# meffmadd/intro-tc-vae

Measured on AMD Instinct MI355X. Metric: images/sec (64x64x3, z=128, bs=64) intro-TC step, higher is better.
Workload: dtype f32 in/out/accumulate, conv products on split-fp16 MFMA (two scaled fp16 planes, 3 products, fp32-class)

## Files before the change

include/itcv_hip.h:

```cpp
#ifndef ITCV_HIP_H
#define ITCV_HIP_H

#include <stddef.h>
#include <stdint.h>

#ifdef __cplusplus
extern "C" {
#endif

#define ITCV_ABI_VERSION 4

int itcv_abi_version(void);
const char* itcv_last_error(void);
int itcv_set_option(const char* name, int value);
int itcv_get_option(const char* name);

int itcv_profile_begin(void);
int itcv_profile_end(void);
int itcv_profile_get(int i, int* code, double* flop, float* ms);
int itcv_profile_clear(void);

size_t itcv_conv2d_packed_weight_elems(int Co, int Ci, int KS, int for_dgrad);
int itcv_conv2d_pack_weight(const float* w, float* wp, int Co, int Ci, int KS, int for_dgrad,
                            void* stream);
// ... 93 lines not shown
                     void* stream);
int itcv_bn_finalize_uv(const double* sums, double count, float eps, float momentum, float* running_mean,
                        float* running_var, int64_t* num_batches_tracked, float* mean, float* rstd, float* unbiased_var,
                        int C, void* stream);
int itcv_bn_eval_stats(const float* running_mean, const float* running_var, float eps, float* mean,
                       float* rstd, int C, void* stream);
int itcv_bn_act_fwd(const float* x, const float* mean, const float* rstd, const float* gamma,
                    const float* beta, const float* skip, float* y, int B, int C, int H, int W,
                    float slope, int pool, void* planes, int ns, size_t plane_stride, void* stream);
int itcv_bn_act_planes_supported(int C, int H, int W, int pool);
int itcv_bn_act_bwd_reduce(const float* x, const float* dy, const float* mean, const float* rstd,
                           const float* gamma, const float* beta, const float* skip, double* dsums,
                           float* dgamma, float* dbeta, int accumulate, int B, int C, int H, int W,
                           float slope, int pool, int up2, void* ws, size_t ws_bytes, void* stream);
int itcv_bn_act_bwd_apply(const float* x, const float* dy, const float* mean, const float* rstd,
                          const float* gamma, const float* beta, const float* skip, const double* dsums,
                          const double* local_dsums, double count, float* dx, float* dskip,
                          float* dgamma, float* dbeta, int accumulate, int B, int C, int H, int W,
                          float slope, int pool, int up2, void* dx_planes, int ns, size_t plane_stride, void* stream);

int itcv_bn_train_fwd(const float* x, const float* gamma, const float* beta, const float* skip, float* y, void* planes,
                      int ns, int B, int C, int H, int W, float slope, int pool, float eps, float momentum,
                      float* running_mean, float* running_var, int64_t* num_batches_tracked, float* mean, float* rstd,
                      void* ws, size_t ws_bytes, size_t plane_stride, const float* tile_stats, int tiles, int tile_pitch,
                      int groups, void* stream);
int itcv_bn_train_fwd_uv(const float* x, const float* gamma, const float* beta, const float* skip, float* y, void* planes,
                         int ns, int B, int C, int H, int W, float slope, int pool, float eps, float momentum,
                         float* running_mean, float* running_var, int64_t* num_batches_tracked, float* mean, float* rstd,
                         float* unbiased_var, void* ws, size_t ws_bytes, size_t plane_stride, const float* tile_stats,
                         int tiles, int tile_pitch, int groups, void* stream);
size_t itcv_bn_replay_desc_bytes(void);
int itcv_bn_replay_desc(void* host_desc, float* running_mean, float* running_var, int64_t* num_batches_tracked,
                        const float* mean, const float* unbiased_var, int C, int groups, float momentum, int block0);
int itcv_bn_replay_many(const void* dev_table, int n, int total_blocks, void* stream);
int itcv_bn_replay_max_descs(void);
int itcv_bn_train_bwd(const float* x, const float* dy, const float* mean, const float* rstd, const float* gamma,
                      const float* beta, const float* skip, double* dsums, float* dx, float* dskip, void* dx_planes,
                      int ns, float* dgamma, float* dbeta, int accumulate, int B, int C, int H, int W, float slope,
                      int pool, int up2, void* ws, size_t ws_bytes, size_t plane_stride, int groups, void* stream);
int itcv_bn_train_bwd_live(const float* x, const float* dy, const float* mean, const float* rstd, const float* gamma,
                           const float* beta, const float* skip, double* dsums, float* dx, float* dskip, void* dx_planes,
                           int ns, float* dgamma, float* dbeta, int accumulate, int B, int C, int H, int W, float slope,
                           int pool, int up2, void* ws, size_t ws_bytes, size_t plane_stride, int groups, int live0,
                           int nlive, void* stream);

#define ITCV_BN_PATH_ONE_BLOCK 0
#define ITCV_BN_PATH_SLICED_FOLD 1
#define ITCV_BN_PATH_SLICED_COMBINE 2
#define ITCV_BN_PATH_FALLBACK 3
#define ITCV_BN_PATH_PER_GROUP 4
#define ITCV_BN_PATH_TILE_STATS 5
int itcv_bn_plan_query(int bwd, int B, int C, int H, int W, int pool, int up2, int groups, int planes, int ns,
                       size_t ws_bytes, int tile_stats, int* path, int* splits);

int itcv_lrelu_fwd(const float* x, float* y, size_t n, float slope, void* stream);
int itcv_lrelu_bwd(const float* x, const float* dy, float* dx, size_t n, float slope, void* stream);
int itcv_sigmoid_fwd(const float* x, float* y, size_t n, void* stream);
int itcv_sigmoid_bwd(const float* y, const float* dy, float* dx, size_t n, void* stream);
int itcv_avgpool2_fwd(const float* x, float* y, int BC, int H, int W, void* stream);
int itcv_avgpool2_bwd(const float* dy, float* dx, int BC, int H, int W, void* stream);
int itcv_upsample2_fwd(const float* x, float* y, int BC, int H, int W, void* stream);
int itcv_upsample2_bwd(const float* dy, float* dx, int BC, int H, int W, void* stream);
int itcv_add(const float* a, const float* b, float* out, size_t n, void* stream);

int itcv_reparam_fwd(const float* mu, const float* logvar, const float* eps, float* z, size_t n,
                     void* stream);
int itcv_reparam_bwd(const float* dz, const float* logvar, const float* eps, float* dmu, float* dlogvar,
                     size_t n, void* stream);
int itcv_kl_rows_fwd(const float* logvar, const float* mu, float* kl, int B, int D, void* stream);
int itcv_kl_rows_bwd(const float* g, const float* logvar, const float* mu, float* dlogvar, float* dmu,
                     int B, int D, void* stream);

#define ITCV_TC_VAR_FROM_ROW 0x1
#define ITCV_TC_EPS_DENSITY 0x2
#define ITCV_TC_WEIGHTED 0x4
#define ITCV_TC_LIVE (ITCV_TC_VAR_FROM_ROW | ITCV_TC_EPS_DENSITY)
size_t itcv_tc_fwd_workspace(int Bl, int Bt, int D);
int itcv_tc_fwd(const float* z, const float* mu_all, const float* logvar, float* prodm, float* logqz,
                float* lse, float* sjoint, int Bl, int Bt, int row_offset, int D, int64_t dataset_size, int flags,
                void* ws, size_t ws_bytes, void* stream);
size_t itcv_tc_bwd_workspace(int Bl, int Bt);
int itcv_tc_bwd(const float* g, const float* z, const float* mu_all, const float* logvar,
                const float* logqz, const float* lse, const float* sjoint, float* dz, float* dmu_all,
                float* dlogvar, int Bl, int Bt, int row_offset, int D, int64_t dataset_size, int flags, void* ws,
                size_t ws_bytes, void* stream);
int itcv_tc_kl_fwd(const float* z, const float* mu_all, const float* logvar, float* out, float* rows, float* prodm,
                   float* logqz, float* lse, float* sjoint, int Bl, int Bt, int row_offset, int D, int64_t dataset_size,
                   float coef_tc, float coef_kl, int reduction, void* ws, size_t ws_bytes, void* stream);
int itcv_tc_kl_bwd(const float* g, const float* z, const float* mu_all, const float* logvar, const float* logqz,
                   const float* lse, const float* sjoint, float* dz, float* dmu_all, float* dlogvar, int Bl, int Bt,
                   int row_offset, int D, int64_t dataset_size, float coef_tc, float coef_kl, int reduction, void* ws,
                   size_t ws_bytes, void* stream);
size_t itcv_tc_full_fwd_workspace(int Bl, int Bt, int D);
int itcv_tc_full_fwd(const float* z, const float* mu_all, const float* logvar_all, int ld, float* out, float* rows,
                     float* comps, float* prodm, float* logqz, float* lse, float* sjoint, float* ivar, int Bl, int Bt,
                     int row_offset, int D, int64_t dataset_size, float alpha, float beta, float gamma, int reduction,
                     void* ws, size_t ws_bytes, void* stream);
size_t itcv_tc_full_bwd_workspace(int Bl, int Bt);
int itcv_tc_full_bwd(const float* g, const float* z, const float* mu_all, const float* logvar_all, int ld,
                     const float* logqz, const float* lse, const float* sjoint, const float* ivar, float* dz, float* dmu_all,
                     float* dlogvar_all, int Bl, int Bt, int row_offset, int D, int64_t dataset_size, float alpha,
                     float beta, float gamma, int reduction, void* ws, size_t ws_bytes, void* stream);
int itcv_kl_loss_fwd(const float* logvar, const float* mu, float* out, int B, int D, int reduction, float scale, void* stream);
int itcv_kl_loss_bwd(const float* g, const float* logvar, const float* mu, float* dlogvar, float* dmu, int B, int D,
                     int reduction, float scale, void* stream);
size_t itcv_dip_kl_workspace(int Bt, int D);
// ... 267 lines not shown
```

intro-tc-vae_amd/csrc/abi.hip:

```cpp
#include "conv_shared.h"

#include <vector>

namespace itcv {
thread_local char g_err[512] = "";

struct ProfRec {
  int code;
  double flop;
  hipEvent_t start, stop;
};
static bool g_prof_on = false;
static std::vector<ProfRec> g_prof;

static thread_local int g_prof_depth = 0;
ProfScope::ProfScope(hipStream_t stream, ProfKind kind, int ks, int bm, int up2, int ns, double flop) : st(stream), slot(-1) {
  if (++g_prof_depth > 1 || !g_prof_on) return;
  ProfRec r;
  r.code = kind | (ks << 4) | (bm << 8) | (up2 << 16) | (ns << 20);
  r.flop = flop;
  if (hipEventCreate(&r.start) != hipSuccess || hipEventCreate(&r.stop) != hipSuccess) return;
  g_prof.push_back(r);
  slot = (int)g_prof.size() - 1;
  g_prof_start = r.start, g_prof_stop = r.stop;
}
ProfScope::~ProfScope() {
  if (--g_prof_depth > 0) return;
  if (slot >= 0 && g_prof_start) {
    (void)hipEventDestroy(g_prof[slot].start);
    (void)hipEventDestroy(g_prof[slot].stop);
    g_prof.pop_back();
  }
  g_prof_start = g_prof_stop = nullptr;
}
thread_local hipEvent_t g_prof_start = nullptr, g_prof_stop = nullptr;
Options g_opt;
extern int g_sw_lds_rows, g_sw_max_blocks;
}

extern "C" {
int itcv_abi_version(void) { return ITCV_ABI_VERSION; }

int itcv_set_option(const char* name, int value) {
  if (!name) return itcv::fail("%s: null option name", "itcv_set_option");
  if (!strcmp(name, "band_m16")) {
    if (value != 0 && value != 1) return itcv::fail("%s: band_m16 takes 0 or 1 (got %lld)", "itcv_set_option", value);
    itcv::g_opt.band_m16 = value;
    return 0;
  }
  if (!strcmp(name, "band_persist_blocks")) {
    if (value < 0 || value > 1024) return itcv::fail("%s: band_persist_blocks takes 0..1024 (got %lld)", "itcv_set_option", value);
    itcv::g_opt.band_persist_blocks = value;
    return 0;
  }
  if (!strcmp(name, "wgrad_m16")) {
    if (value != 0 && value != 1) return itcv::fail("%s: wgrad_m16 takes 0 or 1 (got %lld)", "itcv_set_option", value);
    itcv::g_opt.wgrad_m16 = value;
    return 0;
  }
  if (!strcmp(name, "planes_mfma_waves")) {
    if (value != 4 && value != 8) return itcv::fail("%s: planes_mfma_waves takes 4 or 8 (got %lld)", "itcv_set_option", value);
    itcv::g_opt.planes_mfma_waves = value;
    return 0;
  }
  if (!strcmp(name, "sw_lds_rows")) {
    if (value < 0 || value > 4096) return itcv::fail("%s: sw_lds_rows takes 0..4096 (got %lld)", "itcv_set_option", value);
    itcv::g_sw_lds_rows = value;
    return 0;
  }
  if (!strcmp(name, "sw_max_blocks")) {
    if (value < 0 || value > 1024) return itcv::fail("%s: sw_max_blocks takes 0..1024 (got %lld)", "itcv_set_option", value);
    itcv::g_sw_max_blocks = value;
    return 0;
  }
  return itcv::fail("%s: unknown option", "itcv_set_option");
}
int itcv_get_option(const char* name) {
  if (name && !strcmp(name, "band_m16")) return itcv::g_opt.band_m16;
  if (name && !strcmp(name, "band_persist_blocks")) return itcv::g_opt.band_persist_blocks;
  if (name && !strcmp(name, "wgrad_m16")) return itcv::g_opt.wgrad_m16;
  if (name && !strcmp(name, "planes_mfma_waves")) return itcv::g_opt.planes_mfma_waves;
  if (name && !strcmp(name, "sw_lds_rows")) return itcv::g_sw_lds_rows;
  if (name && !strcmp(name, "sw_max_blocks")) return itcv::g_sw_max_blocks;
  return -1;
}
const char* itcv_last_error(void) { return itcv::g_err; }

int itcv_profile_begin(void) {
  itcv::g_prof.clear();
  itcv::g_prof_on = true;
  return 0;
}
int itcv_profile_end(void) {
  itcv::g_prof_on = false;
  for (auto& r : itcv::g_prof) (void)hipEventSynchronize(r.stop);
  return (int)itcv::g_prof.size();
}
int itcv_profile_get(int i, int* code, double* flop, float* ms) {
  if (i < 0 || i >= (int)itcv::g_prof.size()) return itcv::fail("%s: index out of range", "itcv_profile_get");
  const auto& r = itcv::g_prof[i];
  *code = r.code;
  *flop = r.flop;
  if (hipEventElapsedTime(ms, r.start, r.stop) != hipSuccess) *ms = -1.f;
  return 0;
}
int itcv_profile_clear(void) {
  for (auto& r : itcv::g_prof) {
    (void)hipEventDestroy(r.start);
    (void)hipEventDestroy(r.stop);
  }
  itcv::g_prof.clear();
  return 0;
}
}
```

intro-tc-vae_amd/csrc/norm_act.hip:

```cpp
#include <stdlib.h>

#include <type_traits>

#include "common.h"

namespace itcv {

constexpr int kRedThreads = 256;

__device__ __forceinline__ uint32_t fdiv(uint32_t a, uint32_t d, int sh) { return sh >= 0 ? (a >> sh) : (a / d); }

struct BnGrp {
  size_t xs;
  size_t os;
  size_t dys;
  size_t ps;
  int cs;
  int G;
  int lv0, lvn;
};
__device__ __forceinline__ bool bn_dead(const BnGrp& g, uint32_t group) {
  return g.lvn > 0 && (group < (uint32_t)g.lv0 || group >= (uint32_t)(g.lv0 + g.lvn));
}

// ... 335 lines not shown
      const float mu = p_mu[j], rs = p_rs[j];
      const float sc = p_ga[j] * rs, sh = p_be[j] - mu * sc;
      const size_t bc = (size_t)b * C + c;
      if (POOL == 0) {
        const size_t i = bc * HW + (size_t)pp * 4;
        float4 v = xin[POOL ? 0 : j];
        v.x = v.x * sc + sh, v.y = v.y * sc + sh, v.z = v.z * sc + sh, v.w = v.w * sc + sh;
        if (skip) {
          const float4 k = *reinterpret_cast<const float4*>(skip + i);
          v.x += k.x, v.y += k.y, v.z += k.z, v.w += k.w;
        }
        v.x = lrelu(v.x, slope), v.y = lrelu(v.y, slope), v.z = lrelu(v.z, slope), v.w = lrelu(v.w, slope);
        if (y) *reinterpret_cast<float4*>(y + i) = v;
        o[j][0] = v.x, o[j][1] = v.y, o[j][POOL ? 0 : 2] = v.z, o[j][POOL ? 1 : 3] = v.w;
      } else {
        const uint32_t ho = (pp * 2) / Wo, wo = pp * 2 - ho * Wo;
        const size_t src = bc * HW + (size_t)(2 * ho) * W + 2 * wo;
        const float4 a = *reinterpret_cast<const float4*>(x + src);
        const float4 bb = *reinterpret_cast<const float4*>(x + src + W);
        float v0 = a.x * sc + sh, v1 = a.y * sc + sh, v2 = bb.x * sc + sh, v3 = bb.y * sc + sh;
        float w0 = a.z * sc + sh, w1 = a.w * sc + sh, w2 = bb.z * sc + sh, w3 = bb.w * sc + sh;
        if (skip) {
          const float4 ka = *reinterpret_cast<const float4*>(skip + src);
          const float4 kb = *reinterpret_cast<const float4*>(skip + src + W);
          v0 += ka.x, v1 += ka.y, v2 += kb.x, v3 += kb.y;
          w0 += ka.z, w1 += ka.w, w2 += kb.z, w3 += kb.w;
        }
        const float r0 = 0.25f * (lrelu(v0, slope) + lrelu(v1, slope) + lrelu(v2, slope) + lrelu(v3, slope));
        const float r1 = 0.25f * (lrelu(w0, slope) + lrelu(w1, slope) + lrelu(w2, slope) + lrelu(w3, slope));
        if (y) *reinterpret_cast<float2*>(y + bc * HWo + (size_t)pp * 2) = make_float2(r0, r1);
        o[j][0] = r0, o[j][1] = r1;
      }
    }
    u32x4 chk[PX][NS];
#pragma unroll
    for (int px = 0; px < PX; ++px) {
      float v8[8];
#pragma unroll
      for (int j = 0; j < 8; ++j) v8[j] = o[j][px];
      split8<NS, F16>(v8, chk[px]);
    }
    const uint32_t cidx0 = base + (threadIdx.x & ~63u);
    if (cidx0 + 64 <= total) {
      store_planes_wave<PX, NS>(planes, plane_stride, per_plane, (uint32_t)HWo, cidx0, chk, strips[threadIdx.x >> 6]);
    } else {
#pragma unroll
      for (int px = 0; px < PX; ++px)
#pragma unroll
        for (int p = 0; p < NS; ++p) planes[(size_t)p * plane_stride + (size_t)bc8 * HWo + (size_t)pp * PX + px] = chk[px][p];
    }
  }
}

template <int MODE>
__device__ __forceinline__ float upstream(const float* __restrict__ dy, size_t bc, int h, int w, int H, int W) {
  if (MODE == 0) return dy[bc * H * W + (size_t)h * W + w];
  if (MODE == 1) return 0.25f * dy[bc * (H / 2) * (W / 2) + (size_t)(h >> 1) * (W / 2) + (w >> 1)];
  const size_t base = bc * (size_t)(4 * H * W) + (size_t)(2 * h) * (2 * W) + 2 * w;
  const float2 a = *reinterpret_cast<const float2*>(dy + base);
  const float2 b = *reinterpret_cast<const float2*>(dy + base + 2 * W);
  return (a.x + a.y) + (b.x + b.y);
}

template <int MODE>
__global__ __launch_bounds__(kRedThreads) void bn_bwd_partial(const float* __restrict__ x,
                                                              const float* __restrict__ dy,
                                                              const float* __restrict__ mean,
                                                              const float* __restrict__ rstd,
                                                              const float* __restrict__ gamma,
                                                              const float* __restrict__ beta,
                                                              const float* __restrict__ skip,
                                                              double* __restrict__ part, int B, int C, int H, int W,
                                                              float slope, int splits) {
  __shared__ double scratch[kRedThreads / 64];
  const int c = blockIdx.x, s = blockIdx.y, HW = H * W;
  const size_t total = (size_t)B * HW;
  const size_t chunk = (total + splits - 1) / splits;
  const size_t beg = (size_t)s * chunk, end = beg + chunk < total ? beg + chunk : total;
  const float mu = mean[c], rs = rstd[c], ga = gamma[c], be = beta[c];
  double s1 = 0.0, s2 = 0.0;
  for (size_t i = beg + threadIdx.x; i < end; i += kRedThreads) {
    const size_t b = i / HW;
    const int hw = (int)(i - b * HW), h = hw / W, w = hw - h * W;
    const size_t bc = b * C + c;
    const float xh = (x[bc * HW + hw] - mu) * rs;
    float u = xh * ga + be;
    if (skip) u += skip[bc * HW + hw];
    float g = upstream<MODE>(dy, bc, h, w, H, W);
    if (!(u > 0.f)) g *= slope;
    s1 += (double)g;
    s2 += (double)g * (double)xh;
  }
  s1 = block_sum(s1, scratch);
  s2 = block_sum(s2, scratch);
  if (threadIdx.x == 0) {
    part[((size_t)s * 2 + 0) * C + c] = s1;
    part[((size_t)s * 2 + 1) * C + c] = s2;
  }
}

template <int MODE>
__global__ void bn_bwd_apply_kernel(const float* __restrict__ x, const float* __restrict__ dy,
                                    const float* __restrict__ mean, const float* __restrict__ rstd,
                                    const float* __restrict__ gamma, const float* __restrict__ beta,
                                    const float* __restrict__ skip, const double* __restrict__ dsums, double count,
                                    float* __restrict__ dx, float* __restrict__ dskip, int C, int H, int W,
// ... 503 lines not shown
}

static inline int bn_fmt(int ns) { return ns == ITCV_PLANES_F16X2 ? 2 : (ns == 2 ? 0 : 1); }

static int bn_stats_launch(const BnPlan& p, const float* x, int B, int C, int HW, const BnFinal& f, void* ws, size_t ws_bytes,
                           hipStream_t st, const char* who) {
  ITCV_REQUIRE(!p.ws_need || (ws && ws_bytes >= p.ws_need), who);
  double* part = static_cast<double*>(ws);
  if (p.splits == 1)
    hipLaunchKernelGGL(bn_moments_partial<true>, p.rgrid, dim3(kRedThreads), 0, st, x, part, B, C, HW, 1, ilog2_exact(HW), f,
                       p.grp);
  else
    hipLaunchKernelGGL(bn_moments_partial<false>, p.rgrid, dim3(kRedThreads), 0, st, x, part, B, C, HW, p.splits,
                       ilog2_exact(HW), BnFinal{}, p.grp);
  ITCV_CHECK_LAUNCH(who);
  if (p.splits > 1 && p.path != BnPath::SlicedFold) {
    hipLaunchKernelGGL(bn_combine_finalize_groups_kernel, dim3(cdiv(C, 256)), dim3(256), 0, st, part, p.splits, p.G, f.count,
                       f.eps, f.momentum, f.running_mean, f.running_var, f.nbt, f.mean, f.rstd, f.uvar, C);
    ITCV_CHECK_LAUNCH(who);
  }
  return 0;
}

static int bn_fwd_apply_launch(const BnPlan& p, const float* x, const float* mean, const float* rstd, const float* gamma,
                               const float* beta, const float* skip, float* y, void* planes, int ns, int B, int C, int H, int W,
                               float slope, int pool, const BnStatsIn& fold, hipStream_t st) {
  ITCV_REQUIRE((size_t)B * C * H * W < (1ull << 31), "itcv_bn_act_fwd(tensor < 2^31 elements)");
  if (planes) {
    ITCV_REQUIRE(bn_fmt_ok(ns) && itcv_bn_act_planes_supported(C, H, W, pool), "itcv_bn_act_fwd(planes)");
    pick<2>(pool ? 1 : 0, [&](auto pool_c) {
      pick<3>(bn_fmt(ns), [&](auto fmt_c) {
        pick<2>(fold.part ? 1 : 0, [&](auto stats_c) {
          constexpr int POOL = decltype(pool_c)::value, FMT = decltype(fmt_c)::value;
          constexpr bool STATS = decltype(stats_c)::value != 0;
          launch_timed((bn_act_fwd_planes_kernel<POOL, FMT == 1 ? 3 : 2, STATS, FMT == 2>), p.agrid, dim3(256), 0, st, x, mean,
                       rstd, gamma, beta, skip, y, static_cast<u32x4*>(planes), B, C, H, W, slope, fold, p.pstride, p.grp);
        });
      });
    });
    ITCV_CHECK_LAUNCH("itcv_bn_act_fwd(planes)");
    return 0;
  }
  if (pool) ITCV_REQUIRE(H % 2 == 0 && W % 2 == 0, "itcv_bn_act_fwd(pool)");
  else ITCV_REQUIRE((H * W) % 4 == 0, "itcv_bn_act_fwd(H*W % 4)");
  const size_t nout = pool ? (size_t)B * C * (H / 2) * (W / 2) : (size_t)B * C * H * W;
  pick<2>(pool ? 1 : 0, [&](auto pool_c) {
    hipLaunchKernelGGL(bn_act_fwd_kernel<decltype(pool_c)::value>, p.agrid, dim3(256), 0, st, x, mean, rstd, gamma, beta, skip,
                       y, C, H, W, nout, slope, ilog2_exact(H * W), ilog2_exact(C) >= 0 ? C - 1 : -1);
  });
  ITCV_CHECK_LAUNCH("itcv_bn_act_fwd");
  return 0;
}

static int bn_bwd_reduce_launch(const BnPlan& p, const float* x, const float* dy, const float* mean, const float* rstd,
                                const float* gamma, const float* beta, const float* skip, double* dsums, float* dgamma,
                                float* dbeta, int accumulate, int B, int C, int H, int W, float slope, void* ws, size_t ws_bytes,
                                hipStream_t st, const char* who) {
  if (p.mode == 1) ITCV_REQUIRE(H % 2 == 0 && W % 2 == 0, who);
  ITCV_REQUIRE(!p.ws_need || (ws && ws_bytes >= p.ws_need), who);
  ITCV_REQUIRE(!p.f16 || p.vec, "itcv_bn_train_bwd(fp16 planes need W % 4 == 0)");
  double* part = static_cast<double*>(ws);
  float* mx = p.f16 ? reinterpret_cast<float*>(part + p.part_doubles) : nullptr;
  const bool fused = p.vec && p.splits == 1;
  const BnBwdFinal bf = fused ? BnBwdFinal{dsums, dgamma, dbeta, accumulate} : BnBwdFinal{};
  pick<3>(p.mode, [&](auto mode_c) {
    constexpr int MODE = decltype(mode_c)::value;
    if (!p.vec) {
      hipLaunchKernelGGL(bn_bwd_partial<MODE>, p.rgrid, dim3(kRedThreads), 0, st, x, dy, mean, rstd, gamma, beta, skip, part,
                         B, C, H, W, slope, p.splits);
      return;
    }
    pick<2>(fused ? 1 : 0, [&](auto fused_c) {
      pick<2>(p.f16 ? 1 : 0, [&](auto mx_c) {
        pick<2>(p.grp.lvn > 0 ? 1 : 0, [&](auto live_c) {
          pick<2>(ilog2_exact(W) >= 0 && ilog2_exact(H * W) >= 0 ? 1 : 0, [&](auto p2_c) {
            hipLaunchKernelGGL((bn_bwd_partial_v4<MODE, decltype(fused_c)::value != 0, decltype(mx_c)::value != 0,
                                                  decltype(live_c)::value != 0, decltype(p2_c)::value != 0>),
                               p.rgrid, dim3(kRedThreads), 0, st, x, dy, mean, rstd, gamma, beta, skip, part, B, C, H, W, slope,
                               p.splits, ilog2_exact(W), ilog2_exact(H * W), bf, p.grp, mx, p.nmx);
          });
        });
      });
    });
  });
  ITCV_CHECK_LAUNCH(who);
  if (!fused && p.path != BnPath::SlicedFold) {
    hipLaunchKernelGGL(bn_combine_param_groups_kernel, dim3(cdiv(C, 256)), dim3(256), 0, st, part, dsums, C, p.splits, p.G,
                       dgamma, dbeta, accumulate);
    ITCV_CHECK_LAUNCH(who);
  }
  return 0;
}

static int bn_bwd_apply_launch(const BnPlan& p, const float* x, const float* dy, const float* mean, const float* rstd,
                               const float* gamma, const float* beta, const float* skip, const double* dsums, double count,
                               float* dx, float* dskip, void* dx_planes, int ns, int B, int C, int H, int W, float slope,
                               const BnBwdSumsIn& fold, const float* mx, hipStream_t st) {
  ITCV_REQUIRE(x && dy && mean && rstd && gamma && beta && dsums && (dx || dx_planes) && B > 0 && C > 0 && count > 0,
               "itcv_bn_act_bwd_apply");
  const int wsh = ilog2_exact(W);
  if (dx_planes) {
    ITCV_REQUIRE(bn_fmt_ok(ns) && p.vec && itcv_bn_act_planes_supported(C, H, W, 0), "itcv_bn_act_bwd_apply(planes)");
    if (ns == ITCV_PLANES_F16X2 && !mx)
      return fail("%s: fp16 gradient planes take their scale from the maxima of the reduce pass: use itcv_bn_train_bwd",
                  "itcv_bn_act_bwd_apply");
    pick<3>(p.mode, [&](auto mode_c) {
// ... 104 lines not shown
  ITCV_REQUIRE(x && dy && mean && rstd && gamma && beta && dsums && B > 0 && C > 0, "itcv_bn_act_bwd_reduce");
  ITCV_REQUIRE(!(pool && up2), "itcv_bn_act_bwd_reduce(pool and up2 are exclusive)");
  const BnPlan p = bn_plan(true, B, C, H, W, pool, up2, 1, false, 0, 0, ws ? ws_bytes : 0, false);
  return bn_bwd_reduce_launch(p, x, dy, mean, rstd, gamma, beta, skip, dsums, dgamma, dbeta, accumulate, B, C, H, W, slope, ws,
                              ws_bytes, S(stream), "itcv_bn_act_bwd_reduce");
}

int itcv_bn_act_bwd_apply(const float* x, const float* dy, const float* mean, const float* rstd, const float* gamma,
                          const float* beta, const float* skip, const double* dsums, const double* local_dsums,
                          double count, float* dx, float* dskip, float* dgamma, float* dbeta, int accumulate, int B,
                          int C, int H, int W, float slope, int pool, int up2, void* dx_planes, int ns,
                          size_t plane_stride, void* stream) {
  ITCV_REQUIRE(!(pool && up2), "itcv_bn_act_bwd_apply(pool and up2 are exclusive)");
  const BnPlan p = bn_plan(true, B, C, H, W, pool, up2, 1, dx_planes != nullptr, ns, plane_stride, 0, false);
  if (int e = bn_bwd_apply_launch(p, x, dy, mean, rstd, gamma, beta, skip, dsums, count, dx, dskip, dx_planes, ns, B, C, H, W,
                                  slope, BnBwdSumsIn{}, nullptr, S(stream)))
    return e;
  if (dgamma || dbeta) {
    hipLaunchKernelGGL(bn_param_grad_kernel, dim3(cdiv(C, 256)), dim3(256), 0, S(stream), local_dsums ? local_dsums : dsums,
                       dgamma, dbeta, C, accumulate);
    ITCV_CHECK_LAUNCH("itcv_bn_act_bwd_apply(param grads)");
  }
  return 0;
}

int itcv_bn_train_fwd_uv(const float* x, const float* gamma, const float* beta, const float* skip, float* y, void* planes,
                         int ns, int B, int C, int H, int W, float slope, int pool, float eps, float momentum,
                         float* running_mean, float* running_var, int64_t* num_batches_tracked, float* mean, float* rstd,
                         float* unbiased_var, void* ws, size_t ws_bytes, size_t plane_stride, const float* tile_stats,
                         int tiles, int tile_pitch, int groups, void* stream) {
  ITCV_REQUIRE(x && gamma && beta && mean && rstd && (y || planes) && B > 0 && C > 0 && H > 0 && W > 0, "itcv_bn_train_fwd");
  const double px_out = (double)(groups > 1 ? groups : 1) * B * C * (pool ? H * W / 4 : H * W);
  ProfScope bn_prof(S(stream), kProfBnFwd, ilog2_exact(W) >= 0 ? ilog2_exact(W) : 0, C / 8, pool ? 1 : 0, planes ? ns : 0,
                    (double)(groups > 1 ? groups : 1) * B * C * H * W * 4.0 * (skip ? 2 : 1) + px_out * ((planes ? 4.0 : 0.0) + (y ? 4.0 : 0.0)));
  if (groups > 1) ITCV_REQUIRE(!planes || plane_stride, "itcv_bn_train_fwd(groups need the plane stride of the whole tensor)");
  const BnPlan p = bn_plan(false, B, C, H, W, pool, 0, groups, planes != nullptr, ns, plane_stride, ws ? ws_bytes : 0,
                           tile_stats != nullptr);
  if (p.path == BnPath::PerGroup && planes && ns == ITCV_PLANES_F16X2)
    return fail("%s: fp16 planes need the merged group path (no tile statistics, a workspace of itcv_bn_workspace * groups)",
                "itcv_bn_train_fwd");
  if (p.path == BnPath::PerGroup) {
    const BnGrp& s = p.grp;
    for (int g = 0; g < groups; ++g)
      if (int e = itcv_bn_train_fwd_uv(x + g * s.xs, gamma, beta, skip ? skip + g * s.xs : nullptr, y ? y + g * s.os : nullptr,
                                       planes ? static_cast<u32x4*>(planes) + g * s.ps : nullptr, ns, B, C, H, W, slope, pool,
                                       eps, momentum, running_mean, running_var, num_batches_tracked, mean + (size_t)g * C,
                                       rstd + (size_t)g * C, unbiased_var ? unbiased_var + (size_t)g * C : nullptr, ws,
                                       ws_bytes, plane_stride, tile_stats ? tile_stats + (size_t)g * tiles : nullptr, tiles,
                                       tile_pitch, 1, stream))
        return e;
    return 0;
  }
  const BnFinal f{(double)B * H * W, eps, momentum, running_mean, running_var, num_batches_tracked, mean, rstd, unbiased_var};
  if (p.path == BnPath::TileStats) {
    ITCV_REQUIRE(tiles > 0 && tile_pitch >= tiles, "itcv_bn_train_fwd(tile statistics)");
    hipLaunchKernelGGL(bn_tile_stats_finalize_kernel, dim3(C), dim3(256), 0, S(stream), tile_stats, tiles, tile_pitch, f.count,
                       eps, momentum, running_mean, running_var, num_batches_tracked, mean, rstd, unbiased_var, C);
    ITCV_CHECK_LAUNCH("itcv_bn_train_fwd(tile statistics)");
  } else if (int e = bn_stats_launch(p, x, B, C, H * W, f, ws, ws_bytes, S(stream), "itcv_bn_train_fwd(statistics)")) {
    return e;
  }
  const BnStatsIn fold = p.path == BnPath::SlicedFold
                             ? BnStatsIn{static_cast<const double*>(ws), p.splits, f.count, eps, momentum, running_mean,
                                         running_var, num_batches_tracked, mean, rstd, unbiased_var}
                             : BnStatsIn{};
  return bn_fwd_apply_launch(p, x, mean, rstd, gamma, beta, skip, y, planes, ns, B, C, H, W, slope, pool, fold, S(stream));
}

int itcv_bn_train_fwd(const float* x, const float* gamma, const float* beta, const float* skip, float* y, void* planes,
                      int ns, int B, int C, int H, int W, float slope, int pool, float eps, float momentum,
                      float* running_mean, float* running_var, int64_t* num_batches_tracked, float* mean, float* rstd,
                      void* ws, size_t ws_bytes, size_t plane_stride, const float* tile_stats, int tiles, int tile_pitch,
                      int groups, void* stream) {
  return itcv_bn_train_fwd_uv(x, gamma, beta, skip, y, planes, ns, B, C, H, W, slope, pool, eps, momentum, running_mean,
                              running_var, num_batches_tracked, mean, rstd, nullptr, ws, ws_bytes, plane_stride, tile_stats,
                              tiles, tile_pitch, groups, stream);
}

size_t itcv_bn_replay_desc_bytes(void) { return sizeof(BnReplayDesc); }
int itcv_bn_replay_max_descs(void) { return kBnReplayMaxDesc; }
int itcv_bn_replay_desc(void* host_desc, float* running_mean, float* running_var, int64_t* num_batches_tracked,
                        const float* mean, const float* unbiased_var, int C, int groups, float momentum, int block0) {
  if (!(host_desc && C > 0 && groups >= 1 && block0 >= 0 && momentum >= 0.f && momentum <= 1.f) ||
      (running_mean && !mean) || (running_var && !unbiased_var)) {
    fail("%s: bad argument (descriptor, C > 0, groups >= 1, block0 >= 0, momentum in [0, 1], the saved statistics of every "
         "running buffer given)", "itcv_bn_replay_desc");
    return -1;
  }
  if (!running_mean && !running_var && !num_batches_tracked) return 0;
  BnReplayDesc d;
  memset(&d, 0, sizeof(d));
  d.running_mean = running_mean, d.running_var = running_var, d.nbt = num_batches_tracked;
  d.mean = mean, d.uvar = unbiased_var;
  d.C = C, d.G = groups, d.momentum = momentum, d.block0 = block0;
  memcpy(host_desc, &d, sizeof(d));
  return cdiv(C, 256);
}
int itcv_bn_replay_many(const void* dev_table, int n, int total_blocks, void* stream) {
  ITCV_REQUIRE(dev_table && n > 0 && total_blocks > 0, "itcv_bn_replay_many");
  if (n > kBnReplayMaxDesc)
    return fail("%s: at most %d descriptors per table (itcv_bn_replay_max_descs)", "itcv_bn_replay_many", kBnReplayMaxDesc);
  hipLaunchKernelGGL(bn_replay_many, dim3(total_blocks), dim3(256), 0, S(stream),
                     static_cast<const BnReplayDesc*>(dev_table), n);
  ITCV_CHECK_LAUNCH("itcv_bn_replay_many");
  return 0;
}
// ... 23 lines not shown
  if (p.path == BnPath::PerGroup) {
    const BnGrp& s = p.grp;
    for (int g = 0; g < groups; ++g) {
      if (g < live0 || g >= live0 + nlive) {
        if (hipMemsetAsync(dsums + (size_t)g * 2 * C, 0, (size_t)2 * C * sizeof(double), S(stream)) != hipSuccess)
          return fail("%s: clearing a dead group's sums failed", "itcv_bn_train_bwd_live");
        continue;
      }
      if (int e = itcv_bn_train_bwd(x + g * s.xs, dy + g * s.dys, mean + (size_t)g * C, rstd + (size_t)g * C, gamma, beta,
                                    skip ? skip + g * s.xs : nullptr, dsums + (size_t)g * 2 * C, dx ? dx + g * s.xs : nullptr,
                                    dskip ? dskip + g * s.xs : nullptr,
                                    dx_planes ? static_cast<u32x4*>(dx_planes) + g * s.ps : nullptr, ns, dgamma, dbeta,
                                    (accumulate || g > live0) ? 1 : 0, B, C, H, W, slope, pool, up2, ws, ws_bytes,
                                    plane_stride, 1, stream))
        return e;
    }
    return 0;
  }
  if (p.f16) ITCV_REQUIRE(ws && ws_bytes >= ws_need, "itcv_bn_train_bwd(workspace, fp16 planes)");
  if (int e = bn_bwd_reduce_launch(p, x, dy, mean, rstd, gamma, beta, skip, dsums, dgamma, dbeta, accumulate, B, C, H, W, slope,
                                   ws, ws_bytes, S(stream), "itcv_bn_train_bwd(sums)"))
    return e;
  const BnBwdSumsIn fold = p.path == BnPath::SlicedFold
                               ? BnBwdSumsIn{static_cast<const double*>(ws), p.splits, dsums, dgamma, dbeta, accumulate}
                               : BnBwdSumsIn{};
  const float* mx = p.f16 ? reinterpret_cast<const float*>(static_cast<const double*>(ws) + p.part_doubles) : nullptr;
  return bn_bwd_apply_launch(p, x, dy, mean, rstd, gamma, beta, skip, dsums, (double)B * H * W, dx, dskip, dx_planes, ns, B, C,
                             H, W, slope, fold, mx, S(stream));
}

int itcv_bn_train_bwd(const float* x, const float* dy, const float* mean, const float* rstd, const float* gamma,
                      const float* beta, const float* skip, double* dsums, float* dx, float* dskip, void* dx_planes,
                      int ns, float* dgamma, float* dbeta, int accumulate, int B, int C, int H, int W, float slope,
                      int pool, int up2, void* ws, size_t ws_bytes, size_t plane_stride, int groups, void* stream) {
  return itcv_bn_train_bwd_live(x, dy, mean, rstd, gamma, beta, skip, dsums, dx, dskip, dx_planes, ns, dgamma, dbeta,
                                accumulate, B, C, H, W, slope, pool, up2, ws, ws_bytes, plane_stride, groups, 0,
                                groups > 1 ? groups : 1, stream);
}

static_assert((int)BnPath::OneBlock == ITCV_BN_PATH_ONE_BLOCK && (int)BnPath::SlicedFold == ITCV_BN_PATH_SLICED_FOLD &&
                  (int)BnPath::SlicedCombine == ITCV_BN_PATH_SLICED_COMBINE && (int)BnPath::Fallback == ITCV_BN_PATH_FALLBACK &&
                  (int)BnPath::PerGroup == ITCV_BN_PATH_PER_GROUP && (int)BnPath::TileStats == ITCV_BN_PATH_TILE_STATS,
              "ITCV_BN_PATH_* follow BnPath");

int itcv_bn_plan_query(int bwd, int B, int C, int H, int W, int pool, int up2, int groups, int planes, int ns,
                       size_t ws_bytes, int tile_stats, int* path, int* splits) {
  ITCV_REQUIRE(B > 0 && C > 0 && H > 0 && W > 0, "itcv_bn_plan_query");
  const BnPlan p = bn_plan(bwd != 0, B, C, H, W, pool, up2, groups, planes != 0, ns, 0, ws_bytes, tile_stats != 0);
  if (path) *path = (int)p.path;
  if (splits) *splits = p.splits;
  return 0;
}

#define ITCV_POINTWISE(NAME, KERNEL, N, ...)                                                        \
  do {                                                                                              \
    if ((N) == 0) return 0;                                                                         \
    hipLaunchKernelGGL(KERNEL, dim3(grid_for(N)), dim3(256), 0, S(stream), __VA_ARGS__);            \
    ITCV_CHECK_LAUNCH(NAME);                                                                        \
    return 0;                                                                                       \
  } while (0)

int itcv_lrelu_fwd(const float* x, float* y, size_t n, float slope, void* stream) {
  ITCV_REQUIRE(x && y, "itcv_lrelu_fwd");
  ITCV_POINTWISE("itcv_lrelu_fwd", lrelu_fwd_kernel, n, x, y, n, slope);
}
int itcv_lrelu_bwd(const float* x, const float* dy, float* dx, size_t n, float slope, void* stream) {
  ITCV_REQUIRE(x && dy && dx, "itcv_lrelu_bwd");
  ITCV_POINTWISE("itcv_lrelu_bwd", lrelu_bwd_kernel, n, x, dy, dx, n, slope);
}
int itcv_sigmoid_fwd(const float* x, float* y, size_t n, void* stream) {
  ITCV_REQUIRE(x && y, "itcv_sigmoid_fwd");
  ITCV_POINTWISE("itcv_sigmoid_fwd", sigmoid_fwd_kernel, n, x, y, n);
}
int itcv_sigmoid_bwd(const float* y, const float* dy, float* dx, size_t n, void* stream) {
  ITCV_REQUIRE(y && dy && dx, "itcv_sigmoid_bwd");
  ITCV_POINTWISE("itcv_sigmoid_bwd", sigmoid_bwd_kernel, n, y, dy, dx, n);
}
int itcv_add(const float* a, const float* b, float* out, size_t n, void* stream) {
  ITCV_REQUIRE(a && b && out, "itcv_add");
  ITCV_POINTWISE("itcv_add", add_kernel, n, a, b, out, n);
}
int itcv_avgpool2_fwd(const float* x, float* y, int BC, int H, int W, void* stream) {
  ITCV_REQUIRE(x && y && BC > 0 && H > 0 && W > 0 && H % 2 == 0 && W % 2 == 0, "itcv_avgpool2_fwd");
  const size_t n = (size_t)BC * (H / 2) * (W / 2);
  ITCV_POINTWISE("itcv_avgpool2_fwd", avgpool2_fwd_kernel, n, x, y, H, W, n);
}
int itcv_avgpool2_bwd(const float* dy, float* dx, int BC, int H, int W, void* stream) {
  ITCV_REQUIRE(dy && dx && BC > 0 && H > 0 && W > 0 && H % 2 == 0 && W % 2 == 0, "itcv_avgpool2_bwd");
  const size_t n = (size_t)BC * H * W;
  ITCV_POINTWISE("itcv_avgpool2_bwd", avgpool2_bwd_kernel, n, dy, dx, H, W, n);
}
int itcv_upsample2_fwd(const float* x, float* y, int BC, int H, int W, void* stream) {
  ITCV_REQUIRE(x && y && BC > 0 && H > 0 && W > 0, "itcv_upsample2_fwd");
  const size_t n = (size_t)BC * H * W * 4;
  ITCV_POINTWISE("itcv_upsample2_fwd", upsample2_fwd_kernel, n, x, y, H, W, n);
}
int itcv_upsample2_bwd(const float* dy, float* dx, int BC, int H, int W, void* stream) {
  ITCV_REQUIRE(dy && dx && BC > 0 && H > 0 && W > 0, "itcv_upsample2_bwd");
  const size_t n = (size_t)BC * H * W;
  ITCV_POINTWISE("itcv_upsample2_bwd", upsample2_bwd_kernel, n, dy, dx, H, W, n);
}

}
```

Baseline: 4424.

## Fuse BN forward statistics and apply into one LDS-resident launch

Adds a single-kernel batch-norm training forward path for small layers. One block per group of eight channels stages the whole channel slice in LDS, reduces mean and variance there, finalizes the running stats, then applies normalization, skip, leaky-ReLU, optional pooling and the split-fp16 plane packing from LDS. This removes the separate statistics launch and the second global read of x. It is enabled by default when the slice fits in 128 KB of LDS. The cost is a grid of only C/8 blocks, which may leave much of the GPU idle.

```diff
diff --git a/include/itcv_hip.h b/include/itcv_hip.h
--- a/include/itcv_hip.h
+++ b/include/itcv_hip.h
@@ -169,6 +169,7 @@
 #define ITCV_BN_PATH_TILE_STATS 5
 int itcv_bn_plan_query(int bwd, int B, int C, int H, int W, int pool, int up2, int groups, int planes, int ns,
                        size_t ws_bytes, int tile_stats, int* path, int* splits);
+int itcv_bn_fwd_one_launch_supported(int B, int C, int H, int W, int pool, int groups, int planes, int ns);
 
 int itcv_lrelu_fwd(const float* x, float* y, size_t n, float slope, void* stream);
 int itcv_lrelu_bwd(const float* x, const float* dy, float* dx, size_t n, float slope, void* stream);
diff --git a/intro-tc-vae_amd/csrc/abi.hip b/intro-tc-vae_amd/csrc/abi.hip
--- a/intro-tc-vae_amd/csrc/abi.hip
+++ b/intro-tc-vae_amd/csrc/abi.hip
@@ -36,6 +36,7 @@
 thread_local hipEvent_t g_prof_start = nullptr, g_prof_stop = nullptr;
 Options g_opt;
 extern int g_sw_lds_rows, g_sw_max_blocks;
+extern int g_bn_fwd_one_launch;
 }
 
 extern "C" {
@@ -73,6 +74,11 @@
     itcv::g_sw_max_blocks = value;
     return 0;
   }
+  if (!strcmp(name, "bn_fwd_one_launch")) {
+    if (value != 0 && value != 1) return itcv::fail("%s: bn_fwd_one_launch takes 0 or 1 (got %lld)", "itcv_set_option", value);
+    itcv::g_bn_fwd_one_launch = value;
+    return 0;
+  }
   return itcv::fail("%s: unknown option", "itcv_set_option");
 }
 int itcv_get_option(const char* name) {
@@ -82,6 +88,7 @@
   if (name && !strcmp(name, "planes_mfma_waves")) return itcv::g_opt.planes_mfma_waves;
   if (name && !strcmp(name, "sw_lds_rows")) return itcv::g_sw_lds_rows;
   if (name && !strcmp(name, "sw_max_blocks")) return itcv::g_sw_max_blocks;
+  if (name && !strcmp(name, "bn_fwd_one_launch")) return itcv::g_bn_fwd_one_launch;
   return -1;
 }
 const char* itcv_last_error(void) { return itcv::g_err; }
diff --git a/intro-tc-vae_amd/csrc/norm_act.hip b/intro-tc-vae_amd/csrc/norm_act.hip
--- a/intro-tc-vae_amd/csrc/norm_act.hip
+++ b/intro-tc-vae_amd/csrc/norm_act.hip
@@ -411,6 +411,186 @@
   }
 }
 
+constexpr size_t kOneLaunchBytes = 128 * 1024;
+constexpr int kOneThreads = 512, kOneTeams = kOneThreads / kRedThreads, kOneTeamCh = 8 / kOneTeams;
+static_assert(kOneLaunchBytes / (8 * 4 * 4) <= (size_t)kOneThreads * 2, "two trips of the block cover the chunk's pixels");
+__host__ __device__ inline bool bn_one_overlay(uint32_t n, int px) {
+  return (size_t)32 * n + (size_t)(kOneThreads / 64) * 64 * px * 16 > 96 * 1024;
+}
+static_assert((96 * 1024 - (kOneThreads / 64) * 64 * 4 * 16) / 32 == 4 * kOneThreads, "no second trip without the overlay");
+static_assert(64 * 4 * 4 <= 4 * kOneThreads, "an overlaid strip (1024 floats) ends below the second trip's first element");
+
+template <int POOL, int NS, bool F16>
+__global__ __launch_bounds__(kOneThreads) void bn_train_fwd_one_kernel(
+    const float* __restrict__ x, const float* __restrict__ gamma, const float* __restrict__ beta,
+    const float* __restrict__ skip, float* __restrict__ y, u32x4* __restrict__ planes, int B, int C, int H, int W,
+    float slope, BnFinal f, size_t plane_stride, BnGrp grp) {
+  extern __shared__ float4 one_lds[];
+  float* xs = reinterpret_cast<float*>(one_lds);
+  __shared__ double scratch[kOneTeams][2 * kOneTeamCh][kRedThreads / 64];
+  __shared__ float s_mean[8], s_rstd[8];
+  if constexpr (F16) {
+    if (blockIdx.x == 0 && threadIdx.x == 0) {
+      ScaleRec* rec = reinterpret_cast<ScaleRec*>(planes + (size_t)NS * plane_stride);
+      rec->scale = 1.f, rec->inv = 1.f, rec->pad[0] = rec->pad[1] = 0.f;
+    }
+  }
+  constexpr int PX = POOL ? 2 : 4;
+  const uint32_t tid = threadIdx.x, team = tid / kRedThreads, t = tid & (kRedThreads - 1), c8 = blockIdx.x;
+  const uint32_t HW = H * W, C8 = C >> 3, n = (uint32_t)B * HW;
+  const uint32_t Ho = POOL ? H / 2 : H, Wo = POOL ? W / 2 : W, HWo = Ho * Wo;
+  const uint32_t per_plane = HWo / PX, total = (uint32_t)B * per_plane;
+  const uint32_t hw4 = HW >> 2, img4 = 8 * hw4, total4 = (uint32_t)B * img4;
+  u32x4* const strip = reinterpret_cast<u32x4*>(one_lds) +
+                       (bn_one_overlay(n, PX) ? (size_t)(tid >> 6) * (n >> 2) : (size_t)2 * n + (size_t)(tid >> 6) * 64 * PX);
+  const int ngroups = grp.G > 1 ? grp.G : 1;
+  x += (size_t)c8 * 8 * HW;
+  for (int gi = 0; gi < ngroups; ++gi, x += grp.xs, f.mean += grp.cs, f.rstd += grp.cs) {
+    if (gi) {
+      if (skip) skip += grp.xs;
+      if (y) y += grp.os;
+      if (NS) planes += grp.ps;
+      __syncthreads();
+    }
+    auto load_round = [&](const uint32_t q0, auto nk_c) {
+      constexpr int NK = decltype(nk_c)::value;
+      auto ld = [&](int k) {
+        const uint32_t q = q0 + tid + (uint32_t)k * kOneThreads, qq = q < total4 ? q : 0u;
+        const uint32_t b = qq / img4, r = qq - b * img4;
+        return *reinterpret_cast<const float4*>(x + (size_t)b * C * HW + (size_t)r * 4);
+      };
+      auto put = [&](int k, const float4& v) {
+        const uint32_t q = q0 + tid + (uint32_t)k * kOneThreads;
+        if (q < total4) {
+          const uint32_t b = q / img4, r = q - b * img4, j = r / hw4, h4 = r - j * hw4;
+          *reinterpret_cast<float4*>(xs + (size_t)j * n + (size_t)b * HW + (size_t)h4 * 4) = v;
+        }
+      };
+      float4 v0 = ld(0), v1{}, v2{}, v3{}, v4{}, v5{}, v6{}, v7{};
+      if constexpr (NK > 1) v1 = ld(1);
+      if constexpr (NK > 2) v2 = ld(2), v3 = ld(3);
+      if constexpr (NK > 4) v4 = ld(4), v5 = ld(5), v6 = ld(6), v7 = ld(7);
+      put(0, v0);
+      if constexpr (NK > 1) put(1, v1);
+      if constexpr (NK > 2) put(2, v2), put(3, v3);
+      if constexpr (NK > 4) put(4, v4), put(5, v5), put(6, v6), put(7, v7);
+    };
+    for (uint32_t q0 = 0; q0 < total4; q0 += 8 * kOneThreads) {
+      const uint32_t left = total4 - q0;
+      if (left <= 1u * kOneThreads) load_round(q0, std::integral_constant<int, 1>{});
+      else if (left <= 2u * kOneThreads) load_round(q0, std::integral_constant<int, 2>{});
+      else if (left <= 4u * kOneThreads) load_round(q0, std::integral_constant<int, 4>{});
+      else load_round(q0, std::integral_constant<int, 8>{});
+    }
+    __syncthreads();
+    {
+      double s[2 * kOneTeamCh];
+#pragma unroll
+      for (int jj = 0; jj < kOneTeamCh; ++jj) {
+        const float* xc = xs + (size_t)(team * kOneTeamCh + jj) * n;
+        double s1 = 0.0, s2 = 0.0;
+#pragma unroll 4
+        for (uint32_t i = t * 4; i < n; i += kRedThreads * 4) {
+          const float4 v = *reinterpret_cast<const float4*>(xc + i);
+          s1 += ((double)v.x + (double)v.y) + ((double)v.z + (double)v.w);
+          s2 += ((double)v.x * v.x + (double)v.y * v.y) + ((double)v.z * v.z + (double)v.w * v.w);
+        }
+        s[2 * jj] = s1, s[2 * jj + 1] = s2;
+      }
+#pragma unroll
+      for (int k = 0; k < 2 * kOneTeamCh; ++k) s[k] = wave_sum(s[k]);
+      if ((t & 63) == 0) {
+#pragma unroll
+        for (int k = 0; k < 2 * kOneTeamCh; ++k) scratch[team][k][t >> 6] = s[k];
+      }
+      __syncthreads();
+      if ((t & 63) == 0 && (t >> 6) < (uint32_t)kOneTeamCh) {
+        const uint32_t jj = t >> 6, j = team * kOneTeamCh + jj, c = c8 * 8 + j;
+        double s1 = 0, s2 = 0;
+        for (int i = 0; i < kRedThreads / 64; ++i) s1 += scratch[team][2 * jj][i];
+        for (int i = 0; i < kRedThreads / 64; ++i) s2 += scratch[team][2 * jj + 1][i];
+        float mf, rf;
+        bn_finalize(s1, s2, f.count, f.eps, f.momentum, f.running_mean, f.running_var, c, mf, rf,
+                    f.uvar ? f.uvar + (size_t)gi * grp.cs + c : nullptr);
+        f.mean[c] = mf, f.rstd[c] = rf;
+        s_mean[j] = mf, s_rstd[j] = rf;
+        if (c == 0 && f.nbt) f.nbt[0] += 1;
+      }
+      __syncthreads();
+    }
+    for (uint32_t base = 0; base < total; base += kOneThreads) {
+      const uint32_t idx = base + tid;
+      const bool act = idx < total;
+      const uint32_t b = idx / per_plane, pp = idx - b * per_plane;
+      u32x4 chk[PX][NS ? NS : 1];
+      if (act) {
+        float o[8][PX];
+#pragma unroll
+        for (int j = 0; j < 8; ++j) {
+          const int c = c8 * 8 + j;
+          const float mu = s_mean[j], rs = s_rstd[j];
+          const float sc = gamma[c] * rs, sh = beta[c] - mu * sc;
+          const size_t bc = (size_t)b * C + c;
+          const float* xc = xs + (size_t)j * n + (size_t)b * HW;
+          if (POOL == 0) {
+            const size_t i = bc * HW + (size_t)pp * 4;
+            float4 v = *reinterpret_cast<const float4*>(xc + (size_t)pp * 4);
+            v.x = v.x * sc + sh, v.y = v.y * sc + sh, v.z = v.z * sc + sh, v.w = v.w * sc + sh;
+            if (skip) {
+              const float4 k = *reinterpret_cast<const float4*>(skip + i);
+              v.x += k.x, v.y += k.y, v.z += k.z, v.w += k.w;
+            }
+            v.x = lrelu(v.x, slope), v.y = lrelu(v.y, slope), v.z = lrelu(v.z, slope), v.w = lrelu(v.w, slope);
+            if (y) *reinterpret_cast<float4*>(y + i) = v;
+            o[j][0] = v.x, o[j][1] = v.y, o[j][POOL ? 0 : 2] = v.z, o[j][POOL ? 1 : 3] = v.w;
+          } else {
+            const uint32_t ho = (pp * 2) / Wo, wo = pp * 2 - ho * Wo;
+            const size_t loc = (size_t)(2 * ho) * W + 2 * wo, src = bc * HW + loc;
+            const float4 a = *reinterpret_cast<const float4*>(xc + loc);
+            const float4 bb = *reinterpret_cast<const float4*>(xc + loc + W);
+            float v0 = a.x * sc + sh, v1 = a.y * sc + sh, v2 = bb.x * sc + sh, v3 = bb.y * sc + sh;
+            float w0 = a.z * sc + sh, w1 = a.w * sc + sh, w2 = bb.z * sc + sh, w3 = bb.w * sc + sh;
+            if (skip) {
+              const float4 ka = *reinterpret_cast<const float4*>(skip + src);
+              const float4 kb = *reinterpret_cast<const float4*>(skip + src + W);
+              v0 += ka.x, v1 += ka.y, v2 += kb.x, v3 += kb.y;
+              w0 += ka.z, w1 += ka.w, w2 += kb.z, w3 += kb.w;
+            }
+            const float r0 = 0.25f * (lrelu(v0, slope) + lrelu(v1, slope) + lrelu(v2, slope) + lrelu(v3, slope));
+            const float r1 = 0.25f * (lrelu(w0, slope) + lrelu(w1, slope) + lrelu(w2, slope) + lrelu(w3, slope));
+            if (y) *reinterpret_cast<float2*>(y + bc * HWo + (size_t)pp * 2) = make_float2(r0, r1);
+            o[j][0] = r0, o[j][1] = r1;
+          }
+        }
+        if constexpr (NS > 0) {
+#pragma unroll
+          for (int px = 0; px < PX; ++px) {
+            float v8[8];
+#pragma unroll
+            for (int j = 0; j < 8; ++j) v8[j] = o[j][px];
+            split8<NS, F16>(v8, chk[px]);
+          }
+        }
+      }
+      if constexpr (NS > 0) {
+        __syncthreads();
+        if (act) {
+          const uint32_t cidx0 = base + (tid & ~63u);
+          if (cidx0 + 64 <= total) {
+            store_planes_wave<PX, NS>(planes + (size_t)c8 * HWo, plane_stride, per_plane, C8 * HWo, cidx0, chk, strip);
+          } else {
+#pragma unroll
+            for (int px = 0; px < PX; ++px)
+#pragma unroll
+              for (int p = 0; p < NS; ++p)
+                planes[(size_t)p * plane_stride + ((size_t)b * C8 + c8) * HWo + (size_t)pp * PX + px] = chk[px][p];
+          }
+        }
+      }
+    }
+  }
+}
+
 template <int MODE>
 __device__ __forceinline__ float upstream(const float* __restrict__ dy, size_t bc, int h, int w, int H, int W) {
   if (MODE == 0) return dy[bc * H * W + (size_t)h * W + w];
@@ -1020,6 +1200,42 @@
   return 0;
 }
 
+int g_bn_fwd_one_launch = 1;
+static bool bn_fwd_one_ok(const BnPlan& p, int B, int C, int H, int W, int pool, bool planes) {
+  const bool path_ok = planes ? p.path == BnPath::OneBlock : (p.path == BnPath::Fallback && p.splits == 1 && p.G == 1);
+  return path_ok && itcv_bn_act_planes_supported(C, H, W, pool) && (size_t)p.G * B * C * H * W < (1ull << 31) &&
+         (size_t)8 * B * H * W * sizeof(float) <= kOneLaunchBytes;
+}
+
+static int bn_fwd_one_launch(const BnPlan& p, const float* x, const float* gamma, const float* beta, const float* skip,
+                             float* y, void* planes, int ns, int B, int C, int H, int W, float slope, int pool,
+                             const BnFinal& f, hipStream_t st) {
+  const uint32_t n = (uint32_t)B * H * W;
+  const int px = pool ? 2 : 4;
+  const size_t lds = (size_t)32 * n + (planes && !bn_one_overlay(n, px) ? (size_t)(kOneThreads / 64) * 64 * px * 16 : 0);
+  pick<2>(pool ? 1 : 0, [&](auto pool_c) {
+    pick<4>(planes ? 1 + bn_fmt(ns) : 0, [&](auto fmt_c) {
+      constexpr int POOL = decltype(pool_c)::value, FMT = decltype(fmt_c)::value;
+      constexpr auto kernel = bn_train_fwd_one_kernel<POOL, FMT == 0 ? 0 : (FMT == 2 ? 3 : 2), FMT == 3>;
+      if constexpr (FMT != 0) {
+        launch_lds<kernel>(dim3(C / 8), dim3(kOneThreads), lds, st, x, gamma, beta, skip, y, static_cast<u32x4*>(planes), B, C,
+                           H, W, slope, f, p.pstride, p.grp);
+      } else {
+        static size_t have = 0;
+        if (have < lds) {
+          (void)hipFuncSetAttribute(reinterpret_cast<const void*>(kernel), hipFuncAttributeMaxDynamicSharedMemorySize,
+                                    (int)kOneLaunchBytes);
+          have = kOneLaunchBytes;
+        }
+        hipLaunchKernelGGL(kernel, dim3(C / 8), dim3(kOneThreads), lds, st, x, gamma, beta, skip, y,
+                           static_cast<u32x4*>(nullptr), B, C, H, W, slope, f, p.pstride, p.grp);
+      }
+    });
+  });
+  ITCV_CHECK_LAUNCH("itcv_bn_train_fwd(one launch)");
+  return 0;
+}
+
 static int bn_bwd_reduce_launch(const BnPlan& p, const float* x, const float* dy, const float* mean, const float* rstd,
                                 const float* gamma, const float* beta, const float* skip, double* dsums, float* dgamma,
                                 float* dbeta, int accumulate, int B, int C, int H, int W, float slope, void* ws, size_t ws_bytes,
@@ -1230,6 +1446,10 @@
     return 0;
   }
   const BnFinal f{(double)B * H * W, eps, momentum, running_mean, running_var, num_batches_tracked, mean, rstd, unbiased_var};
+  if (g_bn_fwd_one_launch && bn_fwd_one_ok(p, B, C, H, W, pool, planes != nullptr)) {
+    ITCV_REQUIRE(!p.ws_need || (ws && ws_bytes >= p.ws_need), "itcv_bn_train_fwd(statistics)");
+    return bn_fwd_one_launch(p, x, gamma, beta, skip, y, planes, ns, B, C, H, W, slope, pool, f, S(stream));
+  }
   if (p.path == BnPath::TileStats) {
     ITCV_REQUIRE(tiles > 0 && tile_pitch >= tiles, "itcv_bn_train_fwd(tile statistics)");
     hipLaunchKernelGGL(bn_tile_stats_finalize_kernel, dim3(C), dim3(256), 0, S(stream), tile_stats, tiles, tile_pitch, f.count,
@@ -1359,6 +1579,12 @@
   return 0;
 }
 
+int itcv_bn_fwd_one_launch_supported(int B, int C, int H, int W, int pool, int groups, int planes, int ns) {
+  if (B <= 0 || C <= 0 || H <= 0 || W <= 0) return 0;
+  const BnPlan p = bn_plan(false, B, C, H, W, pool, 0, planes ? groups : 1, planes != 0, ns, 0, ~(size_t)0, false);
+  return bn_fwd_one_ok(p, B, C, H, W, pool, planes != 0) ? 1 : 0;
+}
+
 #define ITCV_POINTWISE(NAME, KERNEL, N, ...)                                                        \
   do {                                                                                              \
     if ((N) == 0) return 0;                                                                         \
```

Result: slower. 4360 (-1.4%).
